# cnmoro/MiniVectorDB

Measured on AMD Instinct MI355X. Metric: queries/sec + p50 latency, brute-force IP kNN, 10M×512 fp32, k=10, higher is better.
Workload: dtype f32; 1 GPU; 10000000 x 512 fp32 corpus (10000000 rows resident per GPU), IP, k=10, nq=1 per step; rows_per_gpu=10000000, dim=512, k=10, nq=1, parallelism=row-sharded x1

## Files before the change

minivectordb_amd/csrc/code8_scan.hpp:

```cpp
#pragma once
#include "scan_kernels.hpp"

namespace mvdb {

typedef int i32x4 __attribute__((ext_vector_type(4)));

struct Code8Margin {
    float alpha, beta;
};
__host__ __device__ inline Code8Margin code8_margin(int d, float qnorm, float qstep, float row_norm_bound) {
    const double u = 5.9604644775390625e-08;
    const double qn = (double)qnorm, B = (double)row_norm_bound;
    const double dq = (double)qstep * sqrt((double)d) * 0.5 * 1.001 + qn * 4.0 * u;
    const double kap = 8.0 * u;
    const double gam = (d + 8) * u / (1.0 - (d + 8) * u);
    const double eta = 2.0 * (d + 16) * u;
    const double up = 1.0 + 9.5367431640625e-07;
    Code8Margin m;
    m.alpha = (float)((qn + dq) * (1.0 + kap) * up);
    m.beta = (float)(B * (dq + kap * (qn + dq) + (gam * (1.0 + eta) + eta) * qn) * up + 1e-30);
    return m;
}
__host__ __device__ inline int code8_qmax(int d) { return d <= 512 ? 32512 : 16256; }

// ... 385 lines not shown
            const int64_t i = base + j * kWave + lane;
            c[j] = i < total ? lists[i] : 0ull;
        }
        if (!have_bar) bar = code8_lists_bar(lists, nlists, k);
        have_bar = true;
#pragma unroll
        for (int j = 0; j < UNROLL; ++j) tk.offer(c[j] >= bar ? c[j] : 0ull);
    }
}
__device__ __forceinline__ void code8_merge_lists(WaveTopK& tk, const uint64_t* lists, int nlists, int k, uint64_t* sh, int nwaves) {
    const int64_t total = (int64_t)nlists * k;
    tk.init(k);
    if (total <= (int64_t)nwaves * kWave * 4)
        code8_offer_lists<2>(tk, lists, nlists, k, nwaves);
    else
        code8_offer_lists<kMergeUnroll>(tk, lists, nlists, k, nwaves);
    code8_block_merge(tk, sh, nwaves);
}
__device__ __forceinline__ float code8_lists_floor(const uint64_t* lists, int nlists, int k, uint64_t* sh, float* word, int nwaves) {
    WaveTopK tk;
    code8_merge_lists(tk, lists, nlists, k, sh, nwaves);
    if (threadIdx.x < kWave) {
        const uint64_t kth = readlane_u64(tk.key, k - 1);
        if (threadIdx.x == 0) *word = kth ? fmaxf(key_score(kth), -3.402823466e+38f) : -3.402823466e+38f;
    }
    __syncthreads();
    return *word;
}

struct Code8ScanArgs {
    const uint8_t* high;
    const uint8_t* low;
    const float2* ar;
    int64_t n;
    int d;
    int hstride;
    const int8_t* qhi;
    const int8_t* qlo;
    const float* par;
    const uint64_t* lists;
    int nlists;
    int k;
    float* floor;
    uint32_t* cand;
    int64_t cap;
    unsigned long long* counter;
    unsigned long long* survivors;
    const uint8_t* front;
    unsigned long long* front_survivors;
    unsigned int* front_calls;
    volatile unsigned long long* front_msum;
    volatile unsigned int* front_mcalls;
    const uint8_t* bit2;
};

template <int M>
__device__ __forceinline__ int lane_xor(int v) {
    if constexpr (M == 1)
        return __builtin_amdgcn_update_dpp(0, v, 0xB1, 0xF, 0xF, false);
    else if constexpr (M == 2)
        return __builtin_amdgcn_update_dpp(0, v, 0x4E, 0xF, 0xF, false);
    else if constexpr (M == 8)
        return __builtin_amdgcn_update_dpp(0, v, 0x128, 0xF, 0xF, false);
    else if constexpr (M == 4 || M == 16)
        return __builtin_amdgcn_ds_swizzle(v, (M << 10) | 0x1F);
    else
        return __shfl_xor(v, M);
}

template <int G, int U, int M = 1>
__device__ __forceinline__ int code8_reduce(int (&T)[U], int t) {
    if constexpr (M < U) {
        constexpr int H = U / (2 * M);
        const bool hi = (t & M) != 0;
#pragma unroll
        for (int j = 0; j < H; ++j) {
            const int send = hi ? T[j] : T[j + H];
            const int keep = hi ? T[j + H] : T[j];
            T[j] = keep + lane_xor<M>(send);
        }
        return code8_reduce<G, U, M * 2>(T, t);
    } else if constexpr (M < G) {
        T[0] += lane_xor<M>(T[0]);
        return code8_reduce<G, U, M * 2>(T, t);
    } else {
        return T[0];
    }
}

typedef int i32x3 __attribute__((ext_vector_type(3), aligned(4)));

template <bool QUAD>
struct Code8Narrow {
    typedef int type;
    static __device__ __forceinline__ int part(int v, int) { return v; }
};
template <>
struct Code8Narrow<true> {
    typedef i32x4 type;
    static __device__ __forceinline__ int part(const i32x4& v, int s) { return v[s]; }
};

template <int G, int U, bool MASKED, int GF = 0, int UF = 0, bool LIFT = false>
__global__ __launch_bounds__(kScanThreads) void code8_scan_kernel(Code8ScanArgs a) {
    constexpr int RPI = kWave / G;
    constexpr int RB = RPI * U;
    constexpr bool FRONT = GF > 0;
    static_assert(U >= 2 && U <= 8 && (U & (U - 1)) == 0 && U <= G, "code8_reduce halves U down to one value inside a row group");
    constexpr bool QUAD = FRONT && !MASKED && GF * 32 * kCode8QuadChunks == G * 16;
    static_assert(!FRONT || (UF >= (QUAD ? 1 : 2) && UF <= 8 && (UF & (UF - 1)) == 0 && UF <= GF && kWave % GF == 0), "the same, for the front form");
    const int lane = threadIdx.x & (kWave - 1);
    const int wave = __builtin_amdgcn_readfirstlane(threadIdx.x >> 6);
    const int t = lane % G;
    const int g = lane / G;
    const bool valid = !MASKED || t * 16 < a.d;

    i32x4 qh = {0, 0, 0, 0}, ql = {0, 0, 0, 0};
    if (valid) {
        qh = *reinterpret_cast<const i32x4*>(a.qhi + t * 16);
        ql = *reinterpret_cast<const i32x4*>(a.qlo + t * 16);
    }
    const float qstep = a.par[0], alpha = a.par[1], beta = a.par[2];
    float floor = 0.f;

    int p3 = 0, n3 = 0;
#pragma unroll
    for (int j = 0; j < 4; ++j) {
#pragma unroll
        for (int b = 0; b < 4; ++b) {
            const int Q = ((qh[j] << (24 - 8 * b)) >> 24) * 256 + ((ql[j] << (24 - 8 * b)) >> 24);
            p3 += Q > 0 ? Q : 0;
            n3 += Q < 0 ? -Q : 0;
        }
    }
#pragma unroll
    for (int m = G / 2; m >= 1; m >>= 1) {
        p3 += __shfl_xor(p3, m);
        n3 += __shfl_xor(n3, m);
    }
    const int p7 = __builtin_amdgcn_readfirstlane(p3) * 7, n7 = __builtin_amdgcn_readfirstlane(n3) * 7;
    p3 = __builtin_amdgcn_readfirstlane(p3) * 3;
    n3 = __builtin_amdgcn_readfirstlane(n3) * 3;

    uint32_t stage = 0;
    int nst = 0;
    const unsigned long long cap = (unsigned long long)a.cap;
    auto flush = [&]() __attribute__((always_inline)) {
        unsigned long long base = 0;
        if (lane == 0) base = atomicAdd(a.counter, (unsigned long long)nst);
        base = readlane_u64(base, 0);
        if (lane < nst && base + (unsigned long long)lane < cap) a.cand[base + lane] = stage;
        nst = 0;
    };
    auto append = [&](uint64_t m, uint32_t row) __attribute__((always_inline)) {
        while (m) {
            const int src = __ffsll((long long)m) - 1;
            m &= m - 1;
            const uint32_t v = (uint32_t)__builtin_amdgcn_readlane((int)row, src);
            if (lane == nst) stage = v;
            if (++nst == kWave) flush();
        }
    };

// ... 41 lines not shown
                e = e < ns1 - 1 ? e : ns1 - 1;
                const uint32_t row = (uint32_t)__shfl((int)srow, e);
                const uint32_t* src = reinterpret_cast<const uint32_t*>(a.low) + (int64_t)row * lstride4 + t;
                if (MASKED)
                    lw[u] = valid ? *src : 0u;
                else
                    lw[u] = *src;
            }
            const int e = base + erow;
            const int ec = e < ns1 - 1 ? e : ns1 - 1;
            const uint32_t row = (uint32_t)__shfl((int)srow, ec);
            const int t6 = __shfl(st6, ec);
            const float2 sr = a.ar[row];
            int T[U];
#pragma unroll
            for (int u = 0; u < U; ++u) {
                uint32_t c[4];
                code8_unpack_low(lw[u], c);
                int hi = 0, lo = 0;
#pragma unroll
                for (int j = 0; j < 4; ++j) {
                    hi = __builtin_amdgcn_sdot4((int)c[j], qh[j], hi, false);
                    lo = __builtin_amdgcn_sdot4((int)c[j], ql[j], lo, false);
                }
                T[u] = hi * 256 + lo;
            }
            epilogue(t6 + code8_reduce<G, U>(T, t), sr, __ballot(t < U && e < ns1), row);
        }
        ns1 = 0;
    };
    auto stage1 = [&](int t6, float2 sr, uint64_t mine, int64_t r) __attribute__((always_inline)) {
        const int tl = (t6 > INT_MIN + n3 ? t6 : INT_MIN + n3) - n3;
        const float su = ((float)(t6 + p3) * qstep) * sr.x;
        const float sl = ((float)tl * qstep) * sr.x;
        float m = fmaf(alpha, sr.y, beta);
        m = fmaf(fmaxf(fabsf(su), fabsf(sl)) + m, 2.4e-7f, m);
        const float ub = su + m;
        uint64_t pass = __ballot(!(ub < floor)) & mine;
        while (pass) {
            const int src = __ffsll((long long)pass) - 1;
            pass &= pass - 1;
            const uint32_t v = (uint32_t)__builtin_amdgcn_readlane((int)r, src);
            const int w = __builtin_amdgcn_readlane(t6, src);
            if (lane == ns1) {
                srow = v;
                st6 = w;
            }
            if (++ns1 == kWave) refine();
        }
    };

    const int64_t nwaves_total = (int64_t)gridDim.x * kScanWaves;
    const int64_t gw = (int64_t)blockIdx.x * kScanWaves + wave;
    __shared__ uint64_t sh[(kScanWaves - 1) * kWave];
    __shared__ float sfloor;

    if constexpr (FRONT) {
        constexpr int RPF = kWave / GF;
        constexpr int RBF = RPF * UF;
        const int tf = lane % GF;
        const int gf = lane / GF;
        const bool validf = !MASKED || tf * 32 < a.d;
        constexpr int NC = QUAD ? kCode8QuadChunks : 1;
        typedef typename Code8Narrow<QUAD>::type narrow_t;
        i32x4 fh[NC][2], fl[NC][2];
#pragma unroll
        for (int s = 0; s < NC; ++s) {
#pragma unroll
            for (int i = 0; i < 2; ++i) {
                fh[s][i] = i32x4{0, 0, 0, 0};
                fl[s][i] = i32x4{0, 0, 0, 0};
                if (validf) {
                    fh[s][i] = *reinterpret_cast<const i32x4*>(a.qhi + (tf * NC + s) * 32 + 16 * i);
                    fl[s][i] = *reinterpret_cast<const i32x4*>(a.qlo + (tf * NC + s) * 32 + 16 * i);
                }
            }
        }
        int uef = 0;
#pragma unroll
        for (int m = 1, h = UF / 2; m < UF; m <<= 1, h >>= 1) uef += (tf & m) ? h : 0;
        const int erowf = uef * RPF + gf;
        const uint64_t elanesf = __ballot(tf < UF);

        if (blockIdx.x == 0 && threadIdx.x == 0) {
            const unsigned int calls = atomicAdd(a.front_calls, 1u);
            const unsigned long long sum = atomicAdd(a.front_survivors, 0ull);
            if (a.front_msum) {
                *a.front_msum = sum;
                *a.front_mcalls = calls;
            }
        }

        auto scores0 = [&](const i32x4 (&xw)[UF][NC], const narrow_t (&xn)[UF], int (&T)[UF]) {
#pragma unroll
            for (int u = 0; u < UF; ++u) {
                int hi = 0, lo = 0;
#pragma unroll
                for (int s = 0; s < NC; ++s) {
                    const uint32_t f[5] = {(uint32_t)xw[u][s].x, (uint32_t)xw[u][s].y, (uint32_t)xw[u][s].z, (uint32_t)xw[u][s].w,
                                           (uint32_t)Code8Narrow<QUAD>::part(xn[u], s)};
                    uint32_t c[8];
                    code8_front_unpack_chunk(f, c);
#pragma unroll
                    for (int j = 0; j < 8; ++j) {
                        hi = __builtin_amdgcn_sdot4((int)c[j], fh[s][j >> 2][j & 3], hi, false);
                        lo = __builtin_amdgcn_sdot4((int)c[j], fl[s][j >> 2][j & 3], lo, false);
                    }
// ... 22 lines not shown
                    else
                        x[u] = *src;
                }
                const int e = base + erow;
                const int ec = e < ns0 - 1 ? e : ns0 - 1;
                const uint32_t row = (uint32_t)__shfl((int)s0row, ec);
                const float2 sr = a.ar[row];
#if defined(MVDB_CODE8_ABLATE_GATHER) && MVDB_CODE8_ABLATE_GATHER == 3
#pragma unroll
                for (int u = 0; u < U; ++u) asm volatile("" ::"v"(x[u].x), "v"(x[u].y), "v"(x[u].z));
                asm volatile("" ::"v"(sr.x), "v"(sr.y));
                continue;
#endif
                int T[U];
                scores(x, T);
                stage1(code8_reduce<G, U>(T, t), sr, __ballot(t < U && e < ns0), row);
            }
            ns0 = 0;
        };
        int st5 = 0;
        float sta = 0.f, str = 0.f;
        auto lift_load = [&](int base) __attribute__((always_inline)) {
            int e = base + gf;
            e = e < ns0 - 1 ? e : ns0 - 1;
            const uint32_t row = (uint32_t)__shfl((int)s0row, e);
            const narrow_t* src = reinterpret_cast<const narrow_t*>(a.bit2 + (int64_t)row * code8_bit2_stride(a.d) + tf * (NC * 4));
            if (MASKED) return validf ? *src : narrow_t{};
            return *src;
        };
        auto lift_use = [&](const narrow_t& w, int base) __attribute__((always_inline)) {
            int hi = 0, lo = 0;
#pragma unroll
            for (int s = 0; s < NC; ++s) {
                const uint32_t word = (uint32_t)Code8Narrow<QUAD>::part(w, s);
#pragma unroll
                for (int j = 0; j < 8; ++j) {
                    const int b2 = (int)code8_bit2_spread(word, j);
                    hi = __builtin_amdgcn_sdot4(b2, fh[s][j >> 2][j & 3], hi, false);
                    lo = __builtin_amdgcn_sdot4(b2, fl[s][j >> 2][j & 3], lo, false);
                }
            }
            int T[1] = {hi * 256 + lo};
            const int tot = code8_reduce<GF, 1>(T, tf);
            const int e = base + gf;
            const int ec = e < ns0 - 1 ? e : ns0 - 1;
            const uint32_t row = (uint32_t)__shfl((int)s0row, ec);
            const int t5 = __shfl(st5, ec);
            const float2 sr = make_float2(__shfl(sta, ec), __shfl(str, ec));
            stage1(t5 + 4 * tot, sr, __ballot(tf == 0 && e < ns0), row);
        };
        auto drain0 = [&]() __attribute__((always_inline)) {
            constexpr int UL = 4;
            nfront += (unsigned long long)ns0;
            for (int base = 0; base < ns0; base += UL * RPF) {
                narrow_t w[UL];
#pragma unroll
                for (int u = 0; u < UL; ++u) w[u] = lift_load(base + u * RPF);
#pragma unroll 1
                for (int at = base; at < ns0 && at < base + UL * RPF; at += RPF) {
                    lift_use(w[0], at);
#pragma unroll
                    for (int u = 0; u + 1 < UL; ++u) w[u] = w[u + 1];
                }
            }
            ns0 = 0;
        };
        auto stage0 = [&](int t5, float2 sr, uint64_t mine, int64_t r) __attribute__((always_inline)) {
            const int tl = (t5 > INT_MIN + n7 ? t5 : INT_MIN + n7) - n7;
            const float su = ((float)(t5 + p7) * qstep) * sr.x;
            const float sl = ((float)tl * qstep) * sr.x;
            float m = fmaf(alpha, sr.y, beta);
            m = fmaf(fmaxf(fabsf(su), fabsf(sl)) + m, 2.4e-7f, m);
            const float ub = su + m;
            uint64_t pass = __ballot(!(ub < floor)) & mine;
            while (pass) {
                const int src = __ffsll((long long)pass) - 1;
                pass &= pass - 1;
                const uint32_t v = (uint32_t)__builtin_amdgcn_readlane((int)r, src);
                if constexpr (LIFT) {
                    const int w = __builtin_amdgcn_readlane(t5, src);
                    const float fa = __uint_as_float((uint32_t)__builtin_amdgcn_readlane((int)__float_as_uint(sr.x), src));
                    const float fr = __uint_as_float((uint32_t)__builtin_amdgcn_readlane((int)__float_as_uint(sr.y), src));
                    if (lane == ns0) {
                        s0row = v;
                        st5 = w;
                        sta = fa;
                        str = fr;
                    }
                    if (++ns0 == kWave) drain0();
                } else {
                    if (lane == ns0) s0row = v;
                    if (++ns0 == kWave) gather0();
                }
            }
        };

        const int nch = a.d / 32;
        const int64_t tile_bytes = (int64_t)RPF * code8_front_stride(a.d);
        const int64_t batch_bytes = (int64_t)UF * tile_bytes;
        constexpr int slab = QUAD ? kWave * 16 : 0;
        const int wide_off = QUAD ? lane * 16 : gf * 16 * nch + tf * 16;
        const int narrow_off = QUAD ? NC * slab + lane * 16 : RPF * 16 * nch + gf * 4 * nch + tf * 4;
        const int64_t nfull = a.n / RBF;
        auto load_tile = [&](const uint8_t* tile, i32x4 (&w)[NC], narrow_t& nr) __attribute__((always_inline)) {
            const narrow_t* ns = reinterpret_cast<const narrow_t*>(tile + narrow_off);
#pragma unroll
            for (int s = 0; s < NC; ++s) {
                const i32x4* ws = reinterpret_cast<const i32x4*>(tile + s * slab + wide_off);
                if (MASKED)
                    w[s] = validf ? __builtin_nontemporal_load(ws) : i32x4{0, 0, 0, 0};
                else
                    w[s] = __builtin_nontemporal_load(ws);
            }
#ifdef MVDB_CODE8_ABLATE
            nr = narrow_t{};
            (void)ns;
#else
            if (MASKED)
                nr = validf ? __builtin_nontemporal_load(ns) : narrow_t{};
            else
                nr = __builtin_nontemporal_load(ns);
#endif
        };
        auto load0 = [&](i32x4 (&xw)[UF][NC], narrow_t (&xn)[UF], float2& sr, int64_t b) {
            const uint8_t* base = a.front + b * batch_bytes;
#pragma unroll
            for (int u = 0; u < UF; ++u) load_tile(base + u * tile_bytes, xw[u], xn[u]);
            sr = a.ar[b * RBF + erowf];
        };
        int64_t b = gw;
        const bool head = b < nfull;
        i32x4 xw0[UF][NC];
        narrow_t xn0[UF];
        float2 sr0 = make_float2(0.f, 0.f);
        if (head) load0(xw0, xn0, sr0, b);
        floor = __uint_as_float((uint32_t)__builtin_amdgcn_readfirstlane(
            (int)__float_as_uint(code8_lists_floor(a.lists, a.nlists, a.k, sh, &sfloor, kScanWaves))));
        if (blockIdx.x == 0 && threadIdx.x == 0) *a.floor = floor;
        if (head) {
            int T[UF];
            scores0(xw0, xn0, T);
            stage0(code8_reduce<GF, UF>(T, tf), sr0, elanesf, b * RBF + erowf);
            b += nwaves_total;
        }
        for (; b < nfull; b += nwaves_total) {
            i32x4 xw[UF][NC];
            narrow_t xn[UF];
            float2 sr;
            load0(xw, xn, sr, b);
            int T[UF];
            scores0(xw, xn, T);
            stage0(code8_reduce<GF, UF>(T, tf), sr, elanesf, b * RBF + erowf);
        }
        if (nfull * RBF < a.n && nfull % nwaves_total == gw) {
            const int64_t last = a.n - 1;
            const int64_t last_tile = last / RPF;
            i32x4 xw[UF][NC];
            narrow_t xn[UF];
#pragma unroll
            for (int u = 0; u < UF; ++u) {
                int64_t tile = nfull * UF + u;
                tile = tile < last_tile ? tile : last_tile;
                load_tile(a.front + tile * tile_bytes, xw[u], xn[u]);
            }
            const int64_t r = nfull * RBF + erowf;
            const float2 sr = a.ar[r < last ? r : last];
            int T[UF];
            scores0(xw, xn, T);
            stage0(code8_reduce<GF, UF>(T, tf), sr, __ballot(tf < UF && r < a.n), r);
        }
        if constexpr (LIFT) {
            if (ns0) drain0();
        } else {
            if (ns0) gather0();
        }
        if (ns1) refine();
        if (nfront && lane == 0) atomicAdd(a.front_survivors, nfront);
        if (nrefined && lane == 0) atomicAdd(a.survivors, nrefined);
        if (nst) flush();
        return;
    }

    const int64_t nfull = a.n / RB;
    const int64_t batch_bytes = (int64_t)RB * a.hstride;
    const int64_t group_bytes = (int64_t)RPI * a.hstride;
    const int lane_off = g * a.hstride + t * 12;

    auto load = [&](i32x3 (&x)[U], float2& sr, int64_t b) {
        const uint8_t* base = a.high + b * batch_bytes + lane_off;
#pragma unroll
        for (int u = 0; u < U; ++u) {
            const i32x3* src = reinterpret_cast<const i32x3*>(base + u * group_bytes);
            if (MASKED)
                x[u] = valid ? __builtin_nontemporal_load(src) : i32x3{0, 0, 0};
            else
                x[u] = __builtin_nontemporal_load(src);
        }
        sr = a.ar[b * RB + erow];
    };
    int64_t b = gw;
    const bool head = b < nfull;
    i32x3 x0[U];
    float2 sr0 = make_float2(0.f, 0.f);
    if (head) load(x0, sr0, b);
    floor = __uint_as_float((uint32_t)__builtin_amdgcn_readfirstlane(
        (int)__float_as_uint(code8_lists_floor(a.lists, a.nlists, a.k, sh, &sfloor, kScanWaves))));
    if (blockIdx.x == 0 && threadIdx.x == 0) *a.floor = floor;
    if (head) {
        int T[U];
        scores(x0, T);
        stage1(code8_reduce<G, U>(T, t), sr0, elanes, b * RB + erow);
        b += nwaves_total;
    }
    for (; b < nfull; b += nwaves_total) {
        i32x3 x[U];
        float2 sr;
        load(x, sr, b);
        int T[U];
        scores(x, T);
        stage1(code8_reduce<G, U>(T, t), sr, elanes, b * RB + erow);
    }
    if (nfull * RB < a.n && nfull % nwaves_total == gw) {
        const int64_t last = a.n - 1;
        i32x3 x[U];
#pragma unroll
        for (int u = 0; u < U; ++u) {
            int64_t r = nfull * RB + (int64_t)u * RPI + g;
            r = r < last ? r : last;
            const i32x3* src = reinterpret_cast<const i32x3*>(a.high + r * (int64_t)a.hstride + t * 12);
            if (MASKED)
                x[u] = valid ? __builtin_nontemporal_load(src) : i32x3{0, 0, 0};
            else
// ... 344 lines not shown
```

minivectordb_amd/csrc/common.hpp:

```cpp
#pragma once
#include <hip/hip_runtime.h>
#include <hip/hip_ext.h>
#include <stdint.h>

#include <cstdarg>
#include <cstdio>
#include <cstdlib>
#include <cstring>
#include <mutex>
#include <string>
#include <type_traits>
#include <vector>

#include "../../include/mvdb.h"

namespace mvdb {

void set_error(const char* fmt, ...);
int fail(int code, const char* fmt, ...);

#define MVDB_HIP(expr)                                                                       \
    do {                                                                                     \
        hipError_t e__ = (expr);                                                             \
        if (e__ != hipSuccess)                                                               \
// ... 43 lines not shown
    else hipLaunchKernelGGL(kern, grid, block, lds, stream, args...);
}
void prof_symbol(const char* label, const char* fmt, ...);
template <typename Launch, typename... Sym>
int profiled_launch(const char* label, hipStream_t stream, Launch launch, Sym... symbol) {
    if constexpr (sizeof...(Sym) > 0) prof_symbol(label, symbol...);
    if constexpr (std::is_invocable_v<Launch, hipEvent_t>) {
        hipEvent_t start = nullptr, stop = nullptr;
        const int slot = prof_open(label, stream, &start, &stop);
        if (start) (void)hipEventRecord(start, stream);
        launch(stop);
        prof_close(slot, stream);
    } else {
        const int slot = prof_begin(label, stream);
        if constexpr (std::is_void_v<decltype(launch())>) launch();
        else MVDB_TRY(launch());
        prof_end(slot, stream);
    }
    MVDB_HIP(hipGetLastError());
    return 0;
}

inline int env_int(const char* name, int dflt) {
    const char* v = getenv(name);
    return v && *v ? atoi(v) : dflt;
}

struct Knobs {
    int scan_blocks_per_cu = 0;
    int mfma_blocks_per_cu = 0;
    int mfma_stage = 16;
    int mfma_ng2 = -1;
    int gemm_scan_min_nq = 104;
    int gemm_scan_blocks_per_cu = 2;
    int split_scan_min_nq = -1;
    bool disable_rescue = false;
    bool disable_tile_skip = false;
    int tile_flags_mode = -1;
    int tile_flag_min_tiles = 12288;
    bool disable_rerun_floor = false;
    int half_phase_growth = 0;
    int half_last_growth = 0;
    bool split_stats = false;
    bool disable_mfma_scan = false, disable_l2_mfma = false, disable_gemm_scan = false, disable_split_scan = false,
         disable_half_scan = false, disable_masked_batch = false,
         disable_l2_cert = false,
         disable_half_shadow = false;
    bool shadow_single_query = false;
    bool code8_single_query = true;
    long long code8_capacity = 32768;
    int code8_front_plane = 1;
    int code8_bit_plane = 1;
    int code8_front_u = 0;
    int range_shared = 0;
    int join_shared = 1;
    long long range_candidates = 0;
    long long distinct_table_bytes = 256ll << 20;
    long long maxsim_table_bytes = 2ll << 30;
    int maxsim_tokens_per_pass = 0;
    int assign_vectors_per_pass = 0;
    int examples_vectors_per_pass = 0;
    long long probe_table_bytes = 256ll << 20;
    int grouped_items_per_cu = 0;
    int grouped_min_batches = 4;
    long long compact_bytes = 512ll << 20;
    bool compact_inplace = true;
    int code8_seed_blocks = 0;
    int code8_seed_threads = 0;
    int code8_rescore_rows = 0;
};
Knobs read_knobs();

int cached_occupancy(const void* kern, int threads, size_t lds, int dflt);
int ensure_dynamic_lds(const void* kern, size_t lds, int device);

extern thread_local std::vector<void*>* tls_retire;
struct RetireScope {
    std::vector<void*>* prev;
    explicit RetireScope(std::vector<void*>* list) : prev(tls_retire) { tls_retire = list; }
    ~RetireScope() { tls_retire = prev; }
};

template <typename T>
struct DevBuf {
    T* p = nullptr;
    size_t cap = 0;
    DevBuf() = default;
    DevBuf(const DevBuf&) = delete;
    DevBuf& operator=(const DevBuf&) = delete;
    ~DevBuf() { release(); }
    int reserve(size_t n) {
        if (n <= cap) return 0;
        if (p) {
            if (tls_retire) tls_retire->push_back((void*)p);
            else (void)hipFree(p);
        }
        p = nullptr;
        cap = 0;
        size_t want = n + n / 4 + 64;
        MVDB_HIP(hipMalloc((void**)&p, want * sizeof(T)));
        cap = want;
        return 0;
    }
    void release() {
        if (p) (void)hipFree(p);
        p = nullptr;
// ... 40 lines not shown
```

minivectordb_amd/csrc/mvdb.hip:

```cpp
#include <algorithm>
#include <cmath>
#include <cstdlib>
#include <atomic>
#include <functional>
#include <map>
#include <memory>
#include <tuple>
#include <vector>
#include <shared_mutex>

#include "common.hpp"
#include "index_state.hpp"
#include "scan_kernels.hpp"
#include "grouped_scan.hpp"
#include "range_scan.hpp"
#include "join_scan.hpp"
#include "mmr_select.hpp"
#include "distinct_select.hpp"
#include "maxsim_scan.hpp"
#include "assign_scan.hpp"
#include "examples_scan.hpp"
#include "boost_scan.hpp"
#include "probe_scan.hpp"
#include "code8_scan.hpp"
#include "scan_mfma_kernels.hpp"
#include "select_kernels.hpp"
#include "half_scan.hpp"
#include "util_kernels.hpp"

using namespace mvdb;

namespace mvdb {

int launch_merge_di_sort(int metric, int nlists, int nq, int k, const float* D, int64_t strideD, const int64_t* I,
                         int64_t strideI, float* Dout, int64_t* Iout, int device, hipStream_t stream);

static thread_local char g_err[512] = "";
thread_local std::vector<void*>* tls_retire = nullptr;

Knobs read_knobs() {
    Knobs k;
    k.scan_blocks_per_cu = env_int("MVDB_SCAN_BLOCKS_PER_CU", 0);
    k.mfma_blocks_per_cu = env_int("MVDB_MFMA_BLOCKS_PER_CU", 0);
    k.mfma_stage = env_int("MVDB_MFMA_STAGE", 16);
    k.mfma_ng2 = env_int("MVDB_MFMA_NG2", -1);
    k.gemm_scan_min_nq = env_int("MVDB_GEMM_SCAN_MIN_NQ", 104);
    k.gemm_scan_blocks_per_cu = env_int("MVDB_GEMM_SCAN_BLOCKS_PER_CU", 2);
    k.split_scan_min_nq = env_int("MVDB_SPLIT_SCAN_MIN_NQ", -1);
    k.half_phase_growth = env_int("MVDB_HALF_PHASE_GROWTH", 0);
    k.half_last_growth = env_int("MVDB_HALF_LAST_GROWTH", 0);
    k.split_stats = env_int("MVDB_SPLIT_STATS", 0) != 0;
    k.disable_mfma_scan = env_int("MVDB_DISABLE_MFMA_SCAN", 0) != 0;
    k.disable_l2_mfma = env_int("MVDB_DISABLE_L2_MFMA", 0) != 0;
    k.disable_gemm_scan = env_int("MVDB_DISABLE_GEMM_SCAN", 0) != 0;
    k.disable_split_scan = env_int("MVDB_DISABLE_SPLIT_SCAN", 0) != 0;
    k.disable_half_scan = env_int("MVDB_DISABLE_HALF_SCAN", 0) != 0;
    k.disable_rerun_floor = env_int("MVDB_DISABLE_RERUN_FLOOR", 0) != 0;
    k.disable_rescue = env_int("MVDB_DISABLE_RESCUE", 0) != 0;
    k.disable_tile_skip = env_int("MVDB_DISABLE_TILE_SKIP", 0) != 0;
    k.tile_flag_min_tiles = env_int("MVDB_TILE_FLAG_MIN_TILES", 12288);
    k.tile_flags_mode = env_int("MVDB_TILE_FLAGS", -1);
    k.disable_masked_batch = env_int("MVDB_DISABLE_MASKED_BATCH", 0) != 0;
    k.disable_l2_cert = env_int("MVDB_DISABLE_L2_CERT", 0) != 0;
    k.disable_half_shadow = env_int("MVDB_DISABLE_HALF_SHADOW", 0) != 0;
    k.shadow_single_query = env_int("MVDB_SHADOW_SINGLE_QUERY", 0) != 0;
    k.grouped_items_per_cu = env_int("MVDB_GROUPED_ITEMS_PER_CU", 0);
    k.grouped_min_batches = std::max(1, env_int("MVDB_GROUPED_MIN_BATCHES", 4));
    if (const char* v = getenv("MVDB_COMPACT_BYTES"))
        if (*v) k.compact_bytes = std::max(1ll, atoll(v));
    k.compact_inplace = env_int("MVDB_COMPACT_INPLACE", 1) != 0;
    k.code8_seed_blocks = env_int("MVDB_CODE8_SEED_BLOCKS", 0);
    k.code8_seed_threads = env_int("MVDB_CODE8_SEED_THREADS", 0);
    k.code8_rescore_rows = env_int("MVDB_CODE8_RESCORE_ROWS", 0);
    k.code8_front_u = env_int("MVDB_CODE8_FRONT_U", 0);
    return k;
}

int cached_occupancy(const void* kern, int threads, size_t lds, int dflt) {
    static std::mutex mu;
    static std::map<std::tuple<const void*, size_t, int, int>, int> cache;
    int dev = 0;
    (void)hipGetDevice(&dev);
    std::lock_guard<std::mutex> lk(mu);
    const auto key = std::make_tuple(kern, lds, threads, dev);
    auto it = cache.find(key);
    if (it != cache.end()) return it->second;
    int nb = 0;
    if (hipOccupancyMaxActiveBlocksPerMultiprocessor(&nb, kern, threads, lds) != hipSuccess || nb <= 0) nb = dflt;
    cache[key] = nb;
    return nb;
}

int ensure_dynamic_lds(const void* kern, size_t lds, int device) {
    if (lds == 0) return 0;
    static std::mutex mu;
    static std::map<std::pair<const void*, int>, size_t> done;
    std::lock_guard<std::mutex> lk(mu);
    size_t& have = done[{kern, device}];
    if (lds > have) {
        MVDB_HIP(hipFuncSetAttribute(kern, hipFuncAttributeMaxDynamicSharedMemorySize, (int)lds));
        have = lds;
    }
    return 0;
}

void set_error(const char* fmt, ...) {
    va_list ap;
    va_start(ap, fmt);
    vsnprintf(g_err, sizeof(g_err), fmt, ap);
    va_end(ap);
}
int fail(int code, const char* fmt, ...) {
    va_list ap;
    va_start(ap, fmt);
    vsnprintf(g_err, sizeof(g_err), fmt, ap);
    va_end(ap);
    return code;
}

int ensure_device(int device) {
    int n = 0;
    hipError_t e = hipGetDeviceCount(&n);
    if (e != hipSuccess || n <= 0)
        return fail(MVDB_ERR_NODEVICE, "no HIP device available (%s); libmvdb has no CPU fallback",
                    e == hipSuccess ? "device count is 0" : hipGetErrorString(e));
    if (device < 0 || device >= n)
        return fail(MVDB_ERR_ARG, "device ordinal %d out of range [0,%d)", device, n);
// ... 1732 lines not shown
        drop();
        return 0;
    }
    if (rows != idx->n) return 0;
    MVDB_TRY(build(idx, idx->n, n_new, idx->mut));
    MVDB_TRY(gather_sample(idx, idx->n + n_new, idx->mut));
    MVDB_HIP(hipStreamSynchronize(idx->mut));
    rows = idx->n + n_new;
    return 0;
}

bool code8_route_ok(const mvdb_index* idx, int nq, int k, const int64_t* rows_dev, const uint64_t* mask_dev, int64_t n) {
    if (nq != 1 || !idx->kn.code8_single_query || idx->kn.shadow_single_query) return false;
    if (idx->metric != MVDB_METRIC_IP || rows_dev || mask_dev || k > kMaxFusedK) return false;
    if (n != idx->n || n < kCode8MinRows || !code8_dim(idx->d) || idx->ld != idx->d) return false;
    if (!(idx->row_norm_bound > 0.f) || !(idx->row_norm_bound < 1.0e30f) || idx->code.failed) return false;
    return true;
}

template <int G_, int U_, bool MASKED_, int SCAN_U_, int SCAN_BLOCKS_, int FRONT_G_, int FRONT_U_, int FRONT_BLOCKS_, bool FRONT_DEFAULT_>
struct Code8Shape {
    static constexpr bool FRONT_DEFAULT = FRONT_DEFAULT_;
    static constexpr int G = G_, U = U_, SCAN_U = SCAN_U_, SCAN_BLOCKS = SCAN_BLOCKS_;
    static constexpr int FRONT_G = FRONT_G_, FRONT_U = FRONT_U_, FRONT_BLOCKS = FRONT_BLOCKS_;
    static constexpr bool MASKED = MASKED_;
};
template <typename Launch>
int with_code8_shape(int d, Launch launch) {
    switch (d) {
        case 384: return launch(Code8Shape<32, 8, true, 8, 4, 16, 8, 2, true>{});
        case 512: return launch(Code8Shape<32, 4, false, 8, 2, code8_front_lanes(512), code8_front_quad(512) ? 2 : 4, code8_front_quad(512) ? 1 : 2, true>{});
        case 1024: return launch(Code8Shape<64, 4, false, 8, 2, 32, 4, 2, false>{});
        default: return fail(MVDB_ERR_ARG, "internal: no int8 prefilter kernel for d = %d", d);
    }
}
template <typename Launch>
int with_code8_exact_shape(int d4, Launch launch) {
    return with_scan_shape(d4, [&](auto shape) {
        if constexpr (code8_shape(decltype(shape)::G, decltype(shape)::C)) return launch(shape);
        else return fail(MVDB_ERR_ARG, "internal: no int8 prefilter kernel for rows of %d 16-byte chunks", d4);
    });
}

bool code8_front_wanted(int option, int d) {
    if (option == 0 || !code8_dim(d) || !code8_front_dim(d)) return false;
    bool dflt = false;
    (void)with_code8_shape(d, [&](auto cs) {
        dflt = decltype(cs)::FRONT_DEFAULT;
        return 0;
    });
    return option >= 2 || dflt;
}

template <int G, int U, bool MASKED, int BLOCKS, int GF = 0, int UF = 0, bool LIFT = false>
int code8_scan_blocks(int64_t n, int device) {
    void (*kern)(Code8ScanArgs) = code8_scan_kernel<G, U, MASKED, GF, UF, LIFT>;
    int per_cu = std::min(cached_occupancy((const void*)kern, kScanThreads, 0, 4), BLOCKS);
    if (kn().scan_blocks_per_cu > 0) per_cu = kn().scan_blocks_per_cu;
    return scan_grid(n, GF > 0 ? (kWave / GF) * UF : (kWave / G) * U, per_cu, device);
}
template <int G, int U, bool MASKED, int BLOCKS, int GF = 0, int UF = 0, bool LIFT = false>
int launch_code8_scan(const Code8ScanArgs& a, int device, hipStream_t stream) {
    void (*kern)(Code8ScanArgs) = code8_scan_kernel<G, U, MASKED, GF, UF, LIFT>;
    const int nblocks = code8_scan_blocks<G, U, MASKED, BLOCKS, GF, UF, LIFT>(a.n, device);
    if constexpr (GF > 0)
        return profiled_launch("ip_scan", stream, [&](hipEvent_t done) { launch_kernel(kern, dim3(nblocks), dim3(kScanThreads), 0, stream, done, a); },
                               "code8_scan_kernel<%d, %d, %s, %d, %d>", G, U, MASKED ? "true" : "false", GF, UF);
    else
        return profiled_launch("ip_scan", stream, [&](hipEvent_t done) { launch_kernel(kern, dim3(nblocks), dim3(kScanThreads), 0, stream, done, a); },
                               "code8_scan_kernel<%d, %d, %s>", G, U, MASKED ? "true" : "false");
}
constexpr double kCode8FrontShare = 0.12, kCode8FrontShareQuad = 0.08;
bool code8_front_serves(const mvdb_index* idx) {
    if (!idx->code.F5.p || !code8_front_wanted(idx->kn.code8_front_plane, idx->d)) return false;
    if (idx->kn.code8_front_plane >= 2) return idx->kn.code8_front_plane == 2;
    const volatile unsigned long long* sum = idx->c8_ctr.mirror<unsigned long long>();
    return !idx->c8_front.suspended_mean(sum ? sum + 2 : nullptr, idx->c8_ctr.mirror() ? idx->c8_ctr.mirror() + 6 : nullptr,
                                         (code8_front_quad(idx->d) ? kCode8FrontShareQuad : kCode8FrontShare) * (double)idx->n);
}

template <int G, int U, bool MASKED>
int launch_code8_seed(const Code8SeedArgs& a, int device, hipStream_t stream, int* nlists) {
    void (*kern)(Code8SeedArgs) = code8_seed_kernel<G, U, MASKED>;
    int threads = kn().code8_seed_threads;
    if (threads != 256 && threads != 512 && threads != 1024) threads = kCode8SeedThreads;
    constexpr int64_t nbatches = kCode8Seed / ((kWave / G) * U);
    const int64_t want = (nbatches + threads / kWave - 1) / (threads / kWave);
    int64_t blocks = kn().code8_seed_blocks > 0 ? kn().code8_seed_blocks : device_cus(device);
    blocks = std::max<int64_t>(1, std::min<int64_t>(std::min<int64_t>(blocks, want), scan_grid_upper_bound(device)));
    *nlists = (int)blocks;
    return profiled_launch("ip_scan_code8_seed", stream, [&](hipEvent_t done) { launch_kernel(kern, dim3((unsigned)blocks), dim3(threads), 0, stream, done, a); },
                           "code8_seed_kernel<%d, %d, %s>", G, U, MASKED ? "true" : "false");
}

template <int G, int C, int U, bool MASKED>
int launch_code8_rescore(const Code8RescoreArgs& a, int device, hipStream_t stream) {
    void (*kern)(Code8RescoreArgs) = code8_rescore_kernel<G, C, U, MASKED>;
    const int64_t want = (a.cap + a.rows_per_block - 1) / a.rows_per_block;
    const int64_t blocks = std::max<int64_t>(1, std::min<int64_t>(want, (int64_t)device_cus(device) * 4));
    return profiled_launch("ip_scan_code8_rescore", stream, [&](hipEvent_t done) { launch_kernel(kern, dim3((unsigned)blocks), dim3(kScanThreads), 0, stream, done, a); },
                           "code8_rescore_kernel<%d, %d, %d, %s>", G, C, U, MASKED ? "true" : "false");
}

int code8_search(const mvdb_index* idx, Workspace* ws, const ScanArgs& a0, int k, int64_t label_offset, float* D_dev, int64_t* I_dev,
                 bool* served) {
    *served = false;
    hipStream_t s = ws->stream;
    const int d = idx->d;
    const int64_t cap = std::max<int64_t>(1, std::min<int64_t>(idx->kn.code8_capacity, kCode8MaxCapacity));
    size_t off = 0;
    auto take = [&](size_t bytes) {
        const size_t at = off;
        off += (bytes + 255) / 256 * 256;
        return at;
    };
    const size_t o_planes = take((size_t)2 * d), o_par = take(16 * sizeof(float)), o_ctr = take(2 * sizeof(unsigned long long)),
                 o_gate = take(sizeof(int)), o_floor = take(sizeof(float)), o_cand = take((size_t)cap * sizeof(uint32_t));
    const size_t cand_keys = (size_t)scan_grid_upper_bound(idx->device) * k;
    const bool capturing = stream_capturing(s);
    if (capturing && (ws->c8.cap < off || ws->cand.cap < cand_keys)) return 0;
    if (idx->c8_route.suspended(idx->c8_ctr.mirror())) return 0;
    if (!idx->code.ensure(idx, s)) return 0;
    MVDB_TRY(ws->c8.reserve(off));
// ... 1 lines not shown
    char* base = ws->c8.p;
    int8_t* qhi = reinterpret_cast<int8_t*>(base + o_planes);
    int8_t* qlo = qhi + d;
    float* par = reinterpret_cast<float*>(base + o_par);
    unsigned long long* counter = reinterpret_cast<unsigned long long*>(base + o_ctr);
    int* active = reinterpret_cast<int*>(counter + 1);
    int* gate = reinterpret_cast<int*>(base + o_gate);
    float* floor = reinterpret_cast<float*>(base + o_floor);
    uint32_t* cand = reinterpret_cast<uint32_t*>(base + o_cand);

    ProfChain chain(s);
    Code8SeedArgs sd;
    sd.scodes = idx->code.samp.p;
    sd.sar = reinterpret_cast<const float2*>(idx->code.samp.p + kCode8Seed * d);
    sd.d = d;
    sd.q = a0.q;
    sd.normalize_q = a0.normalize_q;
    sd.row_norm_bound = idx->row_norm_bound;
    sd.qhi = qhi;
    sd.qlo = qlo;
    sd.par = par;
    sd.counter = counter;
    sd.k = k;
    sd.lists = ws->cand.p;
    int seed_lists = 0;
    MVDB_TRY(with_code8_shape(d, [&](auto cs) {
        using K = decltype(cs);
        return launch_code8_seed<K::G, K::U, K::MASKED>(sd, idx->device, s, &seed_lists);
    }));
    Code8ScanArgs c;
    c.high = idx->code.C8.p;
    c.low = idx->code.low(d);
    c.ar = idx->code.ar.p;
    c.n = idx->n;
    c.d = d;
    c.hstride = code8_high_stride(d);
    c.qhi = qhi;
    c.qlo = qlo;
    c.par = par;
    c.lists = ws->cand.p;
    c.nlists = seed_lists;
    c.k = k;
    c.floor = floor;
    c.cand = cand;
    c.cap = cap;
    c.counter = counter;
    c.survivors = reinterpret_cast<unsigned long long*>(idx->c8_ctr.dev() + 2);
    c.front = idx->code.F5.p;
    c.front_survivors = reinterpret_cast<unsigned long long*>(idx->c8_ctr.dev() + 4);
    c.front_calls = idx->c8_ctr.dev() + 6;
    c.front_msum = idx->c8_ctr.mirror<unsigned long long>() + 2;
    c.front_mcalls = idx->c8_ctr.mirror() + 6;
    c.bit2 = idx->code.B2.p;
    const bool front = code8_front_serves(idx);
    const bool lift = front && idx->code.B2.p && idx->kn.code8_bit_plane && kn().code8_front_u == 0;
    MVDB_TRY(with_code8_shape(d, [&](auto cs) {
        using K = decltype(cs);
        if (!front) return launch_code8_scan<K::G, K::SCAN_U, K::MASKED, K::SCAN_BLOCKS>(c, idx->device, s);
        if (lift) return launch_code8_scan<K::G, K::SCAN_U, K::MASKED, K::FRONT_BLOCKS, K::FRONT_G, K::FRONT_U, true>(c, idx->device, s);
        const int hook = kn().code8_front_u;
        if constexpr (code8_front_quad(K::G * 16) && !K::MASKED) {
            const int fu = hook == 1 || hook == 2 || hook == 4 ? hook : K::FRONT_U;
            if (fu == 1) return launch_code8_scan<K::G, K::SCAN_U, K::MASKED, K::FRONT_BLOCKS, K::FRONT_G, 1>(c, idx->device, s);
            if (fu == 2) return launch_code8_scan<K::G, K::SCAN_U, K::MASKED, K::FRONT_BLOCKS, K::FRONT_G, 2>(c, idx->device, s);
            return launch_code8_scan<K::G, K::SCAN_U, K::MASKED, K::FRONT_BLOCKS, K::FRONT_G, 4>(c, idx->device, s);
        } else {
            const int fu = hook == 4 || hook == 8 ? hook : K::FRONT_U;
            if (fu == 4) return launch_code8_scan<K::G, K::SCAN_U, K::MASKED, K::FRONT_BLOCKS, K::FRONT_G, 4>(c, idx->device, s);
            return launch_code8_scan<K::G, K::SCAN_U, K::MASKED, K::FRONT_BLOCKS, K::FRONT_G, 8>(c, idx->device, s);
        }
    }));
    Code8RescoreArgs r;
    r.X = a0.X;
    r.ld = a0.ld;
    r.d4 = a0.d4;
    r.q = a0.q;
    r.normalize_q = a0.normalize_q;
    r.k = k;
    r.cand = cand;
    r.counter = counter;
    r.cap = cap;
    r.par = par;
    r.rows_per_block = kn().code8_rescore_rows > 0 ? kn().code8_rescore_rows : kCode8RescoreRows;
    r.lists = ws->cand.p;
    r.active = active;
    r.gate = gate;
    r.ctr_dev = idx->c8_ctr.dev();
    r.stats = idx->c8_ctr.mirror();
    MVDB_TRY(with_code8_exact_shape(a0.d4, [&](auto shape) {
        using S = decltype(shape);
        return launch_code8_rescore<S::G, S::C, rescore_u(S::G, S::C), false>(r, idx->device, s);
    }));
    ScanArgs a = a0;
    a.cand = ws->cand.p;
    int nblocks = 0;
    a.rows = nullptr;
    a.n = idx->n;
    a.gate = gate;
    a.gate_lo = 0;
    MVDB_TRY(with_code8_exact_shape(a.d4, [&](auto shape) {
        using S = decltype(shape);
        return launch_scan_kern<S::G, S::C, stream_u(S::G, S::C), 0, kModeTopK, 0, false>(a, 1, idx->device, s, &nblocks, "ip_scan_code8_fallback",
                                                                                            false);
    }));
    Code8FinishArgs f;
    f.lists = ws->cand.p;
    f.gate = gate;
    f.active = active;
    f.fallback_lists = nblocks;
    f.k = k;
    f.label_offset = label_offset;
// ... 3456 lines not shown
```

Before: 1944 queries/s.

## Hand off front-stage survivors to a dedicated consumer wave via LDS ring

Adds a fifth wave per block that drains stage-0 survivors from a per-producer shared-memory ring buffer. The four scan waves push survivors into the ring instead of running the gather/lift drain inline, so their streaming scan is not stalled by irregular gathers. They fall back to the inline path when their ring slice is full. This costs 64KB of LDS for the ring, an extra wave per block, and atomic head/tail synchronisation with sleep-polling, all of which may reduce occupancy. It is enabled by default for the quad lift path. It also adds compile-time ablation hooks for the gather stage.

```diff
diff --git a/minivectordb_amd/csrc/code8_scan.hpp b/minivectordb_amd/csrc/code8_scan.hpp
--- a/minivectordb_amd/csrc/code8_scan.hpp
+++ b/minivectordb_amd/csrc/code8_scan.hpp
@@ -461,6 +461,15 @@
     volatile unsigned long long* front_msum;
     volatile unsigned int* front_mcalls;
     const uint8_t* bit2;
+    int ring;
+};
+
+constexpr int kCode8RingMin = 64, kCode8RingMax = 4096, kCode8RingDefault = 1024;
+struct Code8Ring {
+    i32x4 slot[kCode8RingMax];
+    uint32_t tail[kScanWaves];
+    uint32_t head[kScanWaves];
+    uint32_t done;
 };
 
 template <int M>
@@ -510,14 +519,16 @@
     static __device__ __forceinline__ int part(const i32x4& v, int s) { return v[s]; }
 };
 
-template <int G, int U, bool MASKED, int GF = 0, int UF = 0, bool LIFT = false>
-__global__ __launch_bounds__(kScanThreads) void code8_scan_kernel(Code8ScanArgs a) {
+template <int G, int U, bool MASKED, int GF = 0, int UF = 0, bool LIFT = false, bool HANDOFF = false>
+__global__ __launch_bounds__(kScanThreads + (HANDOFF ? kWave : 0)) void code8_scan_kernel(Code8ScanArgs a) {
     constexpr int RPI = kWave / G;
     constexpr int RB = RPI * U;
     constexpr bool FRONT = GF > 0;
     static_assert(U >= 2 && U <= 8 && (U & (U - 1)) == 0 && U <= G, "code8_reduce halves U down to one value inside a row group");
     constexpr bool QUAD = FRONT && !MASKED && GF * 32 * kCode8QuadChunks == G * 16;
     static_assert(!FRONT || (UF >= (QUAD ? 1 : 2) && UF <= 8 && (UF & (UF - 1)) == 0 && UF <= GF && kWave % GF == 0), "the same, for the front form");
+    static_assert(!HANDOFF || (QUAD && LIFT), "the survivor wave serves the quad front form with the lift");
+    constexpr int NW = kScanWaves + (HANDOFF ? 1 : 0);
     const int lane = threadIdx.x & (kWave - 1);
     const int wave = __builtin_amdgcn_readfirstlane(threadIdx.x >> 6);
     const int t = lane % G;
@@ -665,7 +676,7 @@
 
     const int64_t nwaves_total = (int64_t)gridDim.x * kScanWaves;
     const int64_t gw = (int64_t)blockIdx.x * kScanWaves + wave;
-    __shared__ uint64_t sh[(kScanWaves - 1) * kWave];
+    __shared__ uint64_t sh[(NW - 1) * kWave];
     __shared__ float sfloor;
 
     if constexpr (FRONT) {
@@ -794,10 +805,18 @@
         auto drain0 = [&]() __attribute__((always_inline)) {
             constexpr int UL = 4;
             nfront += (unsigned long long)ns0;
+#if defined(MVDB_CODE8_ABLATE_GATHER) && MVDB_CODE8_ABLATE_GATHER == 2
+            ns0 = 0;
+#endif
             for (int base = 0; base < ns0; base += UL * RPF) {
                 narrow_t w[UL];
 #pragma unroll
                 for (int u = 0; u < UL; ++u) w[u] = lift_load(base + u * RPF);
+#if defined(MVDB_CODE8_ABLATE_GATHER) && MVDB_CODE8_ABLATE_GATHER == 3
+#pragma unroll
+                for (int u = 0; u < UL; ++u) asm volatile("" ::"v"(w[u]));
+                continue;
+#endif
 #pragma unroll 1
                 for (int at = base; at < ns0 && at < base + UL * RPF; at += RPF) {
                     lift_use(w[0], at);
@@ -806,6 +825,29 @@
                 }
             }
             ns0 = 0;
+        };
+        [[maybe_unused]] Code8Ring* rg = nullptr;
+        if constexpr (HANDOFF) {
+            __shared__ Code8Ring ring_store;
+            rg = &ring_store;
+        }
+        [[maybe_unused]] const uint32_t rsub = (uint32_t)a.ring / kScanWaves, rmask = rsub - 1u;
+        [[maybe_unused]] uint32_t mytail = 0u;
+        [[maybe_unused]] uint32_t hd_seen = 0u;
+        [[maybe_unused]] auto ring_put = [&](uint64_t pass, int t5, float2 sr, uint32_t r) __attribute__((always_inline)) {
+            const uint32_t cnt = (uint32_t)__popcll(pass);
+            if (mytail - hd_seen + cnt > rsub) {
+                hd_seen = (uint32_t)__builtin_amdgcn_readfirstlane((int)__hip_atomic_load(&rg->head[wave], __ATOMIC_ACQUIRE, __HIP_MEMORY_SCOPE_WORKGROUP));
+                if (mytail - hd_seen + cnt > rsub) return false;
+            }
+            if ((pass >> lane) & 1ull) {
+                const uint32_t slot = (uint32_t)wave * rsub + ((mytail + (uint32_t)__popcll(pass & ((1ull << lane) - 1ull))) & rmask);
+                rg->slot[slot] = i32x4{(int)r, t5, (int)__float_as_uint(sr.x), (int)__float_as_uint(sr.y)};
+            }
+            mytail += cnt;
+            __builtin_amdgcn_fence(__ATOMIC_RELEASE, "workgroup");
+            if (lane == 0) __hip_atomic_store(&rg->tail[wave], mytail, __ATOMIC_RELEASE, __HIP_MEMORY_SCOPE_WORKGROUP);
+            return true;
         };
         auto stage0 = [&](int t5, float2 sr, uint64_t mine, int64_t r) __attribute__((always_inline)) {
             const int tl = (t5 > INT_MIN + n7 ? t5 : INT_MIN + n7) - n7;
@@ -815,6 +857,9 @@
             m = fmaf(fmaxf(fabsf(su), fabsf(sl)) + m, 2.4e-7f, m);
             const float ub = su + m;
             uint64_t pass = __ballot(!(ub < floor)) & mine;
+            if constexpr (HANDOFF) {
+                if (pass && ring_put(pass, t5, sr, (uint32_t)r)) pass = 0ull;
+            }
             while (pass) {
                 const int src = __ffsll((long long)pass) - 1;
                 pass &= pass - 1;
@@ -871,14 +916,73 @@
             sr = a.ar[b * RBF + erowf];
         };
         int64_t b = gw;
-        const bool head = b < nfull;
+        const bool head = (!HANDOFF || wave < kScanWaves) && b < nfull;
         i32x4 xw0[UF][NC];
         narrow_t xn0[UF];
         float2 sr0 = make_float2(0.f, 0.f);
         if (head) load0(xw0, xn0, sr0, b);
+        if constexpr (HANDOFF) {
+            if (threadIdx.x < kScanWaves) {
+                rg->tail[threadIdx.x] = 0u;
+                rg->head[threadIdx.x] = 0u;
+            }
+            if (threadIdx.x == 0) rg->done = 0u;
+        }
         floor = __uint_as_float((uint32_t)__builtin_amdgcn_readfirstlane(
-            (int)__float_as_uint(code8_lists_floor(a.lists, a.nlists, a.k, sh, &sfloor, kScanWaves))));
+            (int)__float_as_uint(code8_lists_floor(a.lists, a.nlists, a.k, sh, &sfloor, NW))));
         if (blockIdx.x == 0 && threadIdx.x == 0) *a.floor = floor;
+        if constexpr (HANDOFF) {
+            if (wave == kScanWaves) {
+                const uint32_t want = rsub < (uint32_t)kWave ? rsub : (uint32_t)kWave;
+                uint32_t hd[kScanWaves] = {0u, 0u, 0u, 0u};
+                for (;;) {
+                    const uint32_t dn = __hip_atomic_load(&rg->done, __ATOMIC_ACQUIRE, __HIP_MEMORY_SCOPE_WORKGROUP);
+                    uint32_t take[kScanWaves], total = 0u;
+#pragma unroll
+                    for (int w = 0; w < kScanWaves; ++w) {
+                        const uint32_t tl = (uint32_t)__builtin_amdgcn_readfirstlane((int)__hip_atomic_load(&rg->tail[w], __ATOMIC_ACQUIRE, __HIP_MEMORY_SCOPE_WORKGROUP));
+                        const uint32_t av = tl - hd[w], room = (uint32_t)kWave - total;
+                        take[w] = av < room ? av : room;
+                        total += take[w];
+                    }
+                    const bool ended = dn == (uint32_t)kScanWaves;
+                    if (total >= want || (ended && total > 0u)) {
+                        uint32_t o = (uint32_t)lane, at = 0u;
+                        bool found = false;
+#pragma unroll
+                        for (int w = 0; w < kScanWaves; ++w) {
+                            if (!found && o < take[w]) {
+                                at = (uint32_t)w * rsub + ((hd[w] + o) & rmask);
+                                found = true;
+                            }
+                            if (!found) o -= take[w];
+                            hd[w] += take[w];
+                        }
+                        if (found) {
+                            const i32x4 e = rg->slot[at];
+                            s0row = (uint32_t)e.x;
+                            st5 = e.y;
+                            sta = __uint_as_float((uint32_t)e.z);
+                            str = __uint_as_float((uint32_t)e.w);
+                        }
+                        ns0 = (int)total;
+                        __builtin_amdgcn_fence(__ATOMIC_RELEASE, "workgroup");
+                        const uint32_t hmine = lane == 0 ? hd[0] : lane == 1 ? hd[1] : lane == 2 ? hd[2] : hd[3];
+                        if (lane < kScanWaves) __hip_atomic_store(&rg->head[lane], hmine, __ATOMIC_RELEASE, __HIP_MEMORY_SCOPE_WORKGROUP);
+                        drain0();
+                    } else if (ended) {
+                        break;
+                    } else {
+                        __builtin_amdgcn_s_sleep(8);
+                    }
+                }
+                if (ns1) refine();
+                if (nfront && lane == 0) atomicAdd(a.front_survivors, nfront);
+                if (nrefined && lane == 0) atomicAdd(a.survivors, nrefined);
+                if (nst) flush();
+                return;
+            }
+        }
         if (head) {
             int T[UF];
             scores0(xw0, xn0, T);
@@ -920,6 +1024,10 @@
         if (nfront && lane == 0) atomicAdd(a.front_survivors, nfront);
         if (nrefined && lane == 0) atomicAdd(a.survivors, nrefined);
         if (nst) flush();
+        if constexpr (HANDOFF) {
+            __builtin_amdgcn_fence(__ATOMIC_RELEASE, "workgroup");
+            if (lane == 0) __hip_atomic_fetch_add(&rg->done, 1u, __ATOMIC_RELEASE, __HIP_MEMORY_SCOPE_WORKGROUP);
+        }
         return;
     }
 
diff --git a/minivectordb_amd/csrc/common.hpp b/minivectordb_amd/csrc/common.hpp
--- a/minivectordb_amd/csrc/common.hpp
+++ b/minivectordb_amd/csrc/common.hpp
@@ -119,6 +119,8 @@
     int code8_front_plane = 1;
     int code8_bit_plane = 1;
     int code8_front_u = 0;
+    int code8_handoff = 0;
+    int code8_ring = 0;
     int range_shared = 0;
     int join_shared = 1;
     long long range_candidates = 0;
diff --git a/minivectordb_amd/csrc/mvdb.hip b/minivectordb_amd/csrc/mvdb.hip
--- a/minivectordb_amd/csrc/mvdb.hip
+++ b/minivectordb_amd/csrc/mvdb.hip
@@ -73,6 +73,8 @@
     k.code8_seed_threads = env_int("MVDB_CODE8_SEED_THREADS", 0);
     k.code8_rescore_rows = env_int("MVDB_CODE8_RESCORE_ROWS", 0);
     k.code8_front_u = env_int("MVDB_CODE8_FRONT_U", 0);
+    k.code8_handoff = env_int("MVDB_CODE8_HANDOFF", 0);
+    k.code8_ring = env_int("MVDB_CODE8_RING", 0);
     return k;
 }
 
@@ -1911,23 +1913,31 @@
     return option >= 2 || dflt;
 }
 
-template <int G, int U, bool MASKED, int BLOCKS, int GF = 0, int UF = 0, bool LIFT = false>
+template <int G, int U, bool MASKED, int BLOCKS, int GF = 0, int UF = 0, bool LIFT = false, bool HANDOFF = false>
 int code8_scan_blocks(int64_t n, int device) {
-    void (*kern)(Code8ScanArgs) = code8_scan_kernel<G, U, MASKED, GF, UF, LIFT>;
-    int per_cu = std::min(cached_occupancy((const void*)kern, kScanThreads, 0, 4), BLOCKS);
+    void (*kern)(Code8ScanArgs) = code8_scan_kernel<G, U, MASKED, GF, UF, LIFT, HANDOFF>;
+    constexpr int threads = kScanThreads + (HANDOFF ? kWave : 0);
+    int per_cu = std::min(cached_occupancy((const void*)kern, threads, 0, 4), BLOCKS);
     if (kn().scan_blocks_per_cu > 0) per_cu = kn().scan_blocks_per_cu;
     return scan_grid(n, GF > 0 ? (kWave / GF) * UF : (kWave / G) * U, per_cu, device);
 }
-template <int G, int U, bool MASKED, int BLOCKS, int GF = 0, int UF = 0, bool LIFT = false>
+template <int G, int U, bool MASKED, int BLOCKS, int GF = 0, int UF = 0, bool LIFT = false, bool HANDOFF = false>
 int launch_code8_scan(const Code8ScanArgs& a, int device, hipStream_t stream) {
-    void (*kern)(Code8ScanArgs) = code8_scan_kernel<G, U, MASKED, GF, UF, LIFT>;
-    const int nblocks = code8_scan_blocks<G, U, MASKED, BLOCKS, GF, UF, LIFT>(a.n, device);
+    void (*kern)(Code8ScanArgs) = code8_scan_kernel<G, U, MASKED, GF, UF, LIFT, HANDOFF>;
+    constexpr int threads = kScanThreads + (HANDOFF ? kWave : 0);
+    const int nblocks = code8_scan_blocks<G, U, MASKED, BLOCKS, GF, UF, LIFT, HANDOFF>(a.n, device);
     if constexpr (GF > 0)
-        return profiled_launch("ip_scan", stream, [&](hipEvent_t done) { launch_kernel(kern, dim3(nblocks), dim3(kScanThreads), 0, stream, done, a); },
+        return profiled_launch("ip_scan", stream, [&](hipEvent_t done) { launch_kernel(kern, dim3(nblocks), dim3(threads), 0, stream, done, a); },
                                "code8_scan_kernel<%d, %d, %s, %d, %d>", G, U, MASKED ? "true" : "false", GF, UF);
     else
-        return profiled_launch("ip_scan", stream, [&](hipEvent_t done) { launch_kernel(kern, dim3(nblocks), dim3(kScanThreads), 0, stream, done, a); },
+        return profiled_launch("ip_scan", stream, [&](hipEvent_t done) { launch_kernel(kern, dim3(nblocks), dim3(threads), 0, stream, done, a); },
                                "code8_scan_kernel<%d, %d, %s>", G, U, MASKED ? "true" : "false");
+}
+constexpr bool kCode8HandoffDefault = true;
+bool code8_handoff_serves() { return kn().code8_handoff == 2 || (kn().code8_handoff != 1 && kCode8HandoffDefault); }
+int code8_ring_entries() {
+    const int r = kn().code8_ring;
+    return r >= kCode8RingMin && r <= kCode8RingMax && (r & (r - 1)) == 0 ? r : kCode8RingDefault;
 }
 constexpr double kCode8FrontShare = 0.12, kCode8FrontShareQuad = 0.08;
 bool code8_front_serves(const mvdb_index* idx) {
@@ -2035,11 +2045,16 @@
     c.front_msum = idx->c8_ctr.mirror<unsigned long long>() + 2;
     c.front_mcalls = idx->c8_ctr.mirror() + 6;
     c.bit2 = idx->code.B2.p;
+    c.ring = code8_ring_entries();
     const bool front = code8_front_serves(idx);
     const bool lift = front && idx->code.B2.p && idx->kn.code8_bit_plane && kn().code8_front_u == 0;
     MVDB_TRY(with_code8_shape(d, [&](auto cs) {
         using K = decltype(cs);
         if (!front) return launch_code8_scan<K::G, K::SCAN_U, K::MASKED, K::SCAN_BLOCKS>(c, idx->device, s);
+        if constexpr (code8_front_quad(K::G * 16) && !K::MASKED) {
+            if (lift && code8_handoff_serves())
+                return launch_code8_scan<K::G, K::SCAN_U, K::MASKED, K::FRONT_BLOCKS, K::FRONT_G, K::FRONT_U, true, true>(c, idx->device, s);
+        }
         if (lift) return launch_code8_scan<K::G, K::SCAN_U, K::MASKED, K::FRONT_BLOCKS, K::FRONT_G, K::FRONT_U, true>(c, idx->device, s);
         const int hook = kn().code8_front_u;
         if constexpr (code8_front_quad(K::G * 16) && !K::MASKED) {
```

Result: faster. 1981 queries/s, median of 6 (+1.9%).
